# zsummer/zsummerX

Measured on AMD Instinct MI355X. Metric: RC4 GiB/s device-resident (batched session payloads) at 1/2/4/8 MI355X, higher is better.
Workload: dtype u8

## Files before the change

### zsummerx_amd/csrc/zrc4_kernels.hpp

```cpp
#pragma once
#include <hip/hip_runtime.h>
#include <stdint.h>
#include "zrc4_plan.hpp"

namespace zrc4 {

constexpr int kGroupBytes = 256 * 256;

enum : uint32_t {
    kErrSlotRange = 0,
    kErrLdsLayout = 1,
    kErrGroup = 2,
    kErrWords = 4,
};

__device__ __forceinline__ void latch_fault(uint32_t *err, uint32_t kind)
{
    __hip_atomic_store(err + kind, 1u, __ATOMIC_RELAXED, __HIP_MEMORY_SCOPE_SYSTEM);
}

constexpr uint32_t kClaimParts = 64;
struct Claim {
    unsigned long long *word;
    uint32_t epoch;
    const uint32_t *zero;
};

__device__ __forceinline__ unsigned long long claim_part(const Claim &cl, uint32_t g, uint32_t part,
                                                         uint32_t bucket)
{
    return __hip_atomic_exchange(cl.word + (size_t)g * kClaimParts + part,
                                 ((unsigned long long)cl.epoch << 32) | bucket, __ATOMIC_RELAXED,
                                 __HIP_MEMORY_SCOPE_AGENT);
}

__device__ __forceinline__ unsigned long long claim_part_async(const Claim &cl, uint32_t g, uint32_t part,
                                                               uint32_t bucket)
{
    unsigned long long old;
    uint64_t sv;
    const unsigned long long v = ((unsigned long long)cl.epoch << 32) | bucket;
    unsigned long long *addr = cl.word + (size_t)g * kClaimParts + part;
    asm volatile("s_mov_b64 %[sv], exec\n\t"
                 "s_mov_b64 exec, 1\n\t"
                 "global_atomic_swap_x2 %[old], %[a], %[v], off sc0\n\t"
                 "s_mov_b64 exec, %[sv]"
                 : [old] "=&v"(old), [sv] "=&s"(sv)
                 : [a] "v"(addr), [v] "v"(v)
                 : "memory");
    return old;
}

__device__ __forceinline__ unsigned long long claim_part_async_if(const Claim &cl, uint32_t g, uint32_t part,
                                                                  uint32_t bucket, uint32_t pred)
{
    unsigned long long old;
    uint64_t sv;
    const unsigned long long v = ((unsigned long long)cl.epoch << 32) | bucket;
    unsigned long long *addr = cl.word + (size_t)g * kClaimParts + part;
    asm volatile("v_mov_b64 %[old], 0\n\t"
                 "s_cmp_eq_u32 %[p], 0\n\t"
                 "s_cbranch_scc1 CLAIM_SKIP_%=\n\t"
                 "s_mov_b64 %[sv], exec\n\t"
                 "s_mov_b64 exec, 1\n\t"
                 "global_atomic_swap_x2 %[old], %[a], %[v], off sc0\n\t"
                 "s_mov_b64 exec, %[sv]\n\t"
                 "CLAIM_SKIP_%=:"
                 : [old] "=&v"(old), [sv] "=&s"(sv)
                 : [a] "v"(addr), [v] "v"(v), [p] "s"(__builtin_amdgcn_readfirstlane(pred))
                 : "memory", "scc");
    return old;
}

__device__ __forceinline__ void claim_wait(unsigned long long &old)
{
    asm volatile("s_waitcnt vmcnt(0)" : "+v"(old) :: "memory");
}

__device__ __forceinline__ bool claim_lost(const Claim &cl, unsigned long long old)
{
    return (uint32_t)(old >> 32) == cl.epoch;
}

__device__ __forceinline__ bool lds_base_ok(const uint8_t *S, uint32_t *err)
{
    if ((uint32_t)(uintptr_t)S == 0u) return true;
    if (threadIdx.x == 0) latch_fault(err, kErrLdsLayout);
    return false;
}

typedef uint32_t u32x4 __attribute__((ext_vector_type(4)));

__host__ __device__ __forceinline__ uint32_t col_of(uint32_t j)
{
    const uint32_t w = j >> 6, l = j & 63u;
    return ((l & 31u) << 2) | (l >> 5) | ((w & 1u) << 1) | ((w >> 1) << 7);
}

__device__ __forceinline__ uint32_t img_vo(uint32_t j)
{
    return (((j & 127u) >> 3) << 8) | (j & 128u) | ((j & 7u) << 4);
}

#ifndef ZRC4_TIMING
#define ZRC4_TIMING 0
#endif
struct Stamps {
    uint64_t r[4], c[4];
};
__device__ __forceinline__ void stamp(Stamps &s, int i)
{
#if ZRC4_TIMING
    s.r[i] = __builtin_amdgcn_s_memrealtime();
    s.c[i] = __builtin_amdgcn_s_memtime();
#endif
}
constexpr uint32_t kStampBase = 65536u + 16384u;
constexpr uint32_t kStampBytes = 131072u + 16384u + 8192u;
__device__ __forceinline__ void stream_stamp(uint8_t *sink, uint32_t i)
{
#if ZRC4_TIMING
    if ((threadIdx.x & 127u) == 0u && blockIdx.x < 512u && i < 16u) {
        const uint32_t r = blockIdx.x * 2u + (threadIdx.x >> 7);
        uint8_t *b = sink + kStampBase;
        reinterpret_cast<uint64_t *>(b)[r * 16u + i] = __builtin_amdgcn_s_memrealtime();
        if (i == 0u || i == 15u)
            reinterpret_cast<uint64_t *>(b + 131072u)[r * 2u + (i ? 1u : 0u)] = __builtin_amdgcn_s_memtime();
        if (i == 0u) {
            uint32_t hw, xcc;
            asm volatile("s_getreg_b32 %0, hwreg(HW_REG_HW_ID)\n\ts_getreg_b32 %1, hwreg(HW_REG_XCC_ID)"
                         : "=s"(hw), "=s"(xcc));
            uint32_t *o = reinterpret_cast<uint32_t *>(b + 131072u + 16384u) + r * 2u;
            o[0] = hw;
            o[1] = xcc;
        }
    }
#endif
}

__device__ __forceinline__ void stamps_out(const Stamps &s, uint8_t *sink, uint32_t wave)
{
#if ZRC4_TIMING
    if ((threadIdx.x & 63u) == 0u) {
        uint64_t *o = reinterpret_cast<uint64_t *>(sink + ((wave & 1023u) * 64u));
        for (int i = 0; i < 4; ++i) {
            o[i] = s.r[i];
            o[4 + i] = s.c[i];
        }
        uint32_t hw, xcc;
        asm volatile("s_getreg_b32 %0, hwreg(HW_REG_HW_ID)\n\ts_getreg_b32 %1, hwreg(HW_REG_XCC_ID)"
                     : "=s"(hw), "=s"(xcc));
        uint32_t *w = reinterpret_cast<uint32_t *>(sink + 65536u + (wave & 1023u) * 8u);
        w[0] = hw;
        w[1] = xcc;
    }
#endif
}

__device__ __forceinline__ void image_to_lds(uint8_t *lds, const uint8_t *img)
{
    const uint4 *src = reinterpret_cast<const uint4 *>(img);
    uint4 *dst = reinterpret_cast<uint4 *>(lds);
#pragma unroll
    for (int i = 0; i < 16; ++i) dst[i * 256 + threadIdx.x] = src[i * 256 + threadIdx.x];
}

__device__ __forceinline__ void lds_to_image(uint8_t *img, const uint8_t *lds)
{
    const uint4 *src = reinterpret_cast<const uint4 *>(lds);
    uint4 *dst = reinterpret_cast<uint4 *>(img);
#pragma unroll
    for (int i = 0; i < 16; ++i) dst[i * 256 + threadIdx.x] = src[i * 256 + threadIdx.x];
}

__device__ __forceinline__ void gather_column(uint8_t *lds, uint32_t col,
                                              const uint8_t *arena, uint32_t slot)
{
    const uint8_t *img = arena + (size_t)(slot >> 8) * kGroupBytes + col_of(slot & 255u);
    for (int k = 0; k < 256; ++k) lds[(k << 8) | col] = img[k << 8];
}

__device__ __forceinline__ void scatter_column(uint8_t *arena, uint32_t slot,
                                               const uint8_t *lds, uint32_t col)
{
    uint8_t *img = arena + (size_t)(slot >> 8) * kGroupBytes + col_of(slot & 255u);
    for (int k = 0; k < 256; ++k) img[k << 8] = lds[(k << 8) | col];
}

struct Rc4Lane {
    uint32_t x0, a0, ya, ta, x1, col;
};

__device__ __forceinline__ void lane_init(Rc4Lane &st, const uint8_t *S, uint32_t col, uint32_t sxy)
{
    const uint32_t x = sxy & 255u, y = (sxy >> 8) & 255u;
    st.col = col;
    st.x0 = (((x + 1u) & 255u) << 8) | col;
    st.a0 = S[st.x0];
    st.ya = (y << 8) | col;
    st.ta = col;
    st.x1 = col;
}

__device__ __forceinline__ uint16_t lane_xy(const Rc4Lane &st)
{
    return (uint16_t)((((st.x0 >> 8) - 1u) & 255u) | (st.ya & 0xFF00u));
}

__device__ __forceinline__ uint32_t prga_step(uint8_t *S, Rc4Lane &st)
{
    const uint32_t a = st.a0;
    const uint32_t ya = (st.ya & 0xFFu) | ((st.ya + (a << 8)) & 0xFF00u);
    const uint32_t b = S[ya];
    S[ya] = (uint8_t)a;
    const uint32_t xn = (st.x0 & 0xFFu) | ((st.x0 + 256u) & 0xFF00u);
    const uint32_t p = S[xn];
    S[st.x0] = (uint8_t)b;
    const uint32_t k = S[(((a + b) << 8) & 0xFF00u) | st.col];
    st.a0 = p;
    st.x0 = xn;
    st.ya = ya;
    return k;
}

__device__ __forceinline__ uint32_t prga_word(uint8_t *S, Rc4Lane &st)
{
    const uint32_t k0 = prga_step(S, st);
    const uint32_t k1 = prga_step(S, st);
    const uint32_t k2 = prga_step(S, st);
    const uint32_t k3 = prga_step(S, st);
    return k0 | (k1 << 8) | (k2 << 16) | (k3 << 24);
}

__device__ __forceinline__ uint4 xor16(uint8_t *S, Rc4Lane &st, uint4 v)
{
    v.x ^= prga_word(S, st);
    v.y ^= prga_word(S, st);
    v.z ^= prga_word(S, st);
    v.w ^= prga_word(S, st);
    return v;
}

#define ZRC4_CORE(XC, XN, A, P, K)                                                               \
    "v_add_u32_sdwa %[ya], %[ya], %[" #A "] dst_sel:BYTE_1 dst_unused:UNUSED_PRESERVE "          \
    "src0_sel:BYTE_1 src1_sel:BYTE_0\n\t"                                                        \
    "ds_read_u8 %[b], %[ya]\n\t"                                                                 \
    "ds_write_b8 %[ya], %[" #A "]\n\t"                                                           \
    "v_add_u16_e32 %[" #XN "], %[c100], %[" #XC "]\n\t"                                          \
    "ds_read_u8 %[" #P "], %[" #XN "]\n\t"                                                       \
    "s_waitcnt lgkmcnt(2)\n\t"                                                                   \
    "ds_write_b8 %[" #XC "], %[b]\n\t"                                                           \
    "v_add_u32_sdwa %[ta], %[" #A "], %[b] dst_sel:BYTE_1 dst_unused:UNUSED_PRESERVE "           \
    "src0_sel:BYTE_0 src1_sel:BYTE_0\n\t"                                                        \
    "ds_read_u8 %[" #K "], %[ta]\n\t"                                                            \
    "s_waitcnt lgkmcnt(2)\n\t"

#define ZRC4_E ZRC4_CORE(x0, x1, a0, a1, k0)
#define ZRC4_O ZRC4_CORE(x1, x0, a1, a0, k1)

__device__ __forceinline__ void load64(uint4 (&q)[4], const uint4 *p)
{
#pragma unroll
    for (int i = 0; i < 4; ++i) q[i] = p[i];
}

__device__ __forceinline__ uint32_t head_bytes(const uint8_t *msg, uint32_t len)
{
    const uint32_t h = (16u - ((uint32_t)(uintptr_t)msg & 15u)) & 15u;
    return h < len ? h : len;
}

#define ZL_XOR(R, SEL, K)                                                                        \
    "v_xor_b32_sdwa " #R ", " #R ", %[" #K "] dst_sel:" #SEL                                     \
    " dst_unused:UNUSED_PRESERVE src0_sel:" #SEL " src1_sel:BYTE_0\n\t"
#define ZL_MOV(R, SEL, K)                                                                        \
    "v_mov_b32_sdwa " #R ", %[" #K "] dst_sel:" #SEL                                             \
    " dst_unused:UNUSED_PRESERVE src0_sel:BYTE_0\n\t"
#define ZL_W0_(X, D)                                                                             \
    ZRC4_E ZRC4_O X(D, BYTE_0, k0) ZRC4_E X(D, BYTE_1, k1)                                      \
    ZRC4_O X(D, BYTE_2, k0)
#define ZL_W_(X, DP, D)                                                                          \
    ZRC4_E X(DP, BYTE_3, k1) ZRC4_O X(D, BYTE_0, k0)                                            \
    ZRC4_E X(D, BYTE_1, k1) ZRC4_O X(D, BYTE_2, k0)
#define ZL_BLOCK_(X, d0, d1, d2, d3, d4, d5, d6, d7, d8, d9, d10, d11, d12, d13, d14, d15)        \
    ZL_W0_(X, d0) ZL_W_(X, d0, d1) ZL_W_(X, d1, d2) ZL_W_(X, d2, d3) ZL_W_(X, d3, d4)           \
    ZL_W_(X, d4, d5) ZL_W_(X, d5, d6) ZL_W_(X, d6, d7) ZL_W_(X, d7, d8) ZL_W_(X, d8, d9)        \
    ZL_W_(X, d9, d10) ZL_W_(X, d10, d11) ZL_W_(X, d11, d12) ZL_W_(X, d12, d13)                  \
    ZL_W_(X, d13, d14) ZL_W_(X, d14, d15)                                                        \
    "s_waitcnt lgkmcnt(0)\n\t" X(d15, BYTE_3, k1)
#define ZL_BLOCK(...) ZL_BLOCK_(ZL_XOR, __VA_ARGS__)
#define ZL_A0 "v[40:43]"
#define ZL_A1 "v[44:47]"
#define ZL_A2 "v[48:51]"
#define ZL_A3 "v[52:55]"
#define ZL_B0 "v[56:59]"
#define ZL_B1 "v[60:63]"
#define ZL_B2 "v[64:67]"
#define ZL_B3 "v[68:71]"
#define ZL_SRC_DELTA "v_lshl_add_u64 v[90:91], v[90:91], 0, %[dl]\n\t"
#define ZL_PREFETCH_(D, R0, R1, R2, R3)                                                          \
    "s_add_u32 %[i1], %[i], 1\n\t"                                                               \
    "v_cmp_lt_u32_e32 vcc, %[i1], %[nblk]\n\t"                                                   \
    "v_lshl_add_u64 v[90:91], v[88:89], 0, 64\n\t"                                               \
    "v_cndmask_b32_e32 v90, v88, v90, vcc\n\t"                                                   \
    "v_cndmask_b32_e32 v91, v89, v91, vcc\n\t"                                                   \
    D                                                                                            \
    "global_load_dwordx4 " R0 ", v[90:91], off\n\t"                                              \
    "global_load_dwordx4 " R1 ", v[90:91], off offset:16\n\t"                                    \
    "global_load_dwordx4 " R2 ", v[90:91], off offset:32\n\t"                                    \
    "global_load_dwordx4 " R3 ", v[90:91], off offset:48\n\t"
#define ZL_STORE(R0, R1, R2, R3)                                                                 \
    "global_store_dwordx4 v[88:89], " R0 ", off\n\t"                                             \
    "global_store_dwordx4 v[88:89], " R1 ", off offset:16\n\t"                                   \
    "global_store_dwordx4 v[88:89], " R2 ", off offset:32\n\t"                                   \
    "global_store_dwordx4 v[88:89], " R3 ", off offset:48\n\t"                                   \
    "v_lshl_add_u64 v[88:89], v[88:89], 0, 64\n\t"                                               \
    "s_add_u32 %[i], %[i], 1\n\t"
#define ZL_ACTIVE                                                                                \
    "v_cmp_lt_u32_e32 vcc, %[i], %[nblk]\n\t"                                                    \
    "s_and_b64 exec, exec, vcc\n\t"                                                              \
    "s_cbranch_execz ZL_DONE_%=\n\t"
#define ZL_HALF_A_(D)                                                                            \
    ZL_ACTIVE                                                                                    \
    ZL_PREFETCH_(D, ZL_B0, ZL_B1, ZL_B2, ZL_B3)                                                  \
    "s_waitcnt vmcnt(8)\n\t"                                                                     \
    ZL_BLOCK(v40, v41, v42, v43, v44, v45, v46, v47, v48, v49, v50, v51, v52, v53, v54, v55)    \
    ZL_STORE(ZL_A0, ZL_A1, ZL_A2, ZL_A3)
#define ZL_HALF_B_(D)                                                                            \
    ZL_ACTIVE                                                                                    \
    ZL_PREFETCH_(D, ZL_A0, ZL_A1, ZL_A2, ZL_A3)                                                  \
    "s_waitcnt vmcnt(8)\n\t"                                                                     \
    ZL_BLOCK(v56, v57, v58, v59, v60, v61, v62, v63, v64, v65, v66, v67, v68, v69, v70, v71)    \
    ZL_STORE(ZL_B0, ZL_B1, ZL_B2, ZL_B3)
#define ZL_FIRST_(D)                                                                             \
    "s_mov_b32 %[i], 0\n\t"                                                                      \
    ZL_PREFETCH_(D, ZL_B0, ZL_B1, ZL_B2, ZL_B3)                                                  \
    "v_mov_b32 v72, 0\n\tv_mov_b32 v73, 0\n\tv_mov_b32 v74, 0\n\tv_mov_b32 v75, 0\n\t"             \
    "v_mov_b32 v76, 0\n\tv_mov_b32 v77, 0\n\tv_mov_b32 v78, 0\n\tv_mov_b32 v79, 0\n\t"             \
    "v_mov_b32 v80, 0\n\tv_mov_b32 v81, 0\n\tv_mov_b32 v82, 0\n\tv_mov_b32 v83, 0\n\t"             \
    "v_mov_b32 v84, 0\n\tv_mov_b32 v85, 0\n\tv_mov_b32 v86, 0\n\tv_mov_b32 v87, 0\n\t"             \
    ZL_BLOCK(v72, v73, v74, v75, v76, v77, v78, v79, v80, v81, v82, v83, v84, v85, v86, v87)    \
    "s_waitcnt vmcnt(4)\n\t"                                                                     \
    "v_xor_b32_e32 v40, v40, v72\n\tv_xor_b32_e32 v41, v41, v73\n\t"                               \
    "v_xor_b32_e32 v42, v42, v74\n\tv_xor_b32_e32 v43, v43, v75\n\t"                               \
    "v_xor_b32_e32 v44, v44, v76\n\tv_xor_b32_e32 v45, v45, v77\n\t"                               \
    "v_xor_b32_e32 v46, v46, v78\n\tv_xor_b32_e32 v47, v47, v79\n\t"                               \
    "v_xor_b32_e32 v48, v48, v80\n\tv_xor_b32_e32 v49, v49, v81\n\t"                               \
    "v_xor_b32_e32 v50, v50, v82\n\tv_xor_b32_e32 v51, v51, v83\n\t"                               \
    "v_xor_b32_e32 v52, v52, v84\n\tv_xor_b32_e32 v53, v53, v85\n\t"                               \
    "v_xor_b32_e32 v54, v54, v86\n\tv_xor_b32_e32 v55, v55, v87\n\t"                               \
    ZL_STORE(ZL_A0, ZL_A1, ZL_A2, ZL_A3)                                                         \
    "s_branch ZL_MID_%=\n\t"

#define ZL_HALF_A ZL_HALF_A_("")
#define ZL_HALF_B ZL_HALF_B_("")
#define ZL_FIRST ZL_FIRST_("")

__device__ __forceinline__ void crypt_blocks_asm(Rc4Lane &st, uint4 *&p, uint32_t nblk,
                                                 const uint4 (&A)[4])
{
    u32x4 a0 = {A[0].x, A[0].y, A[0].z, A[0].w}, a1 = {A[1].x, A[1].y, A[1].z, A[1].w};
    u32x4 a2 = {A[2].x, A[2].y, A[2].z, A[2].w}, a3 = {A[3].x, A[3].y, A[3].z, A[3].w};
    u32x4 b0, b1, b2, b3, q0, q1, q2, q3;
    uint64_t pa = (uint64_t)(uintptr_t)p, pn, save;
    uint32_t i, i1, b, k0, k1, a1s;
    asm volatile(
        "s_mov_b64 %[save], exec\n\t"
        ZL_FIRST
        "ZL_LOOP_%=:\n\t"
        ZL_HALF_A
        "ZL_MID_%=:\n\t"
        ZL_HALF_B
        "s_branch ZL_LOOP_%=\n\t"
        "ZL_DONE_%=:\n\t"
        "s_mov_b64 exec, %[save]\n\t"
        : [ya] "+v"(st.ya), [ta] "+v"(st.ta), [x0] "+v"(st.x0), [x1] "+v"(st.x1),
          [a0] "+v"(st.a0), [a1] "=&v"(a1s), [b] "=&v"(b), [k0] "=&v"(k0), [k1] "=&v"(k1),
          "+{v[88:89]}"(pa), "=&{v[90:91]}"(pn), [i] "=&s"(i), [i1] "=&s"(i1), [save] "=&s"(save),
          "+{v[40:43]}"(a0), "+{v[44:47]}"(a1), "+{v[48:51]}"(a2), "+{v[52:55]}"(a3),
          "=&{v[56:59]}"(b0), "=&{v[60:63]}"(b1), "=&{v[64:67]}"(b2), "=&{v[68:71]}"(b3),
          "=&{v[72:75]}"(q0), "=&{v[76:79]}"(q1), "=&{v[80:83]}"(q2), "=&{v[84:87]}"(q3)
        : [nblk] "v"(nblk), [c100] "s"(0x100u)
        : "memory", "vcc", "scc");
    p = reinterpret_cast<uint4 *>((uintptr_t)pa);
}

#define ZL_TO_LOOP(TAILWAIT)                                                                     \
    asm volatile(                                                                                \
        "s_mov_b64 %[save], exec\n\t"                                                            \
        ZL_FIRST_(ZL_SRC_DELTA)                                                                  \
        "ZL_LOOP_%=:\n\t"                                                                        \
        ZL_HALF_A_(ZL_SRC_DELTA)                                                                 \
        "ZL_MID_%=:\n\t"                                                                         \
        ZL_HALF_B_(ZL_SRC_DELTA)                                                                 \
        "s_branch ZL_LOOP_%=\n\t"                                                                \
        "ZL_DONE_%=:\n\t"                                                                        \
        "s_mov_b64 exec, %[save]\n\t"                                                            \
        TAILWAIT                                                                                 \
        : [ya] "+v"(st.ya), [ta] "+v"(st.ta), [x0] "+v"(st.x0), [x1] "+v"(st.x1),                \
          [a0] "+v"(st.a0), [a1] "=&v"(a1s), [b] "=&v"(b), [k0] "=&v"(k0), [k1] "=&v"(k1),       \
          "+{v[88:89]}"(pa), "=&{v[90:91]}"(pn), [i] "=&s"(i), [i1] "=&s"(i1), [save] "=&s"(save), \
          "+{v[40:43]}"(a0), "+{v[44:47]}"(a1), "+{v[48:51]}"(a2), "+{v[52:55]}"(a3),            \
          "=&{v[56:59]}"(b0), "=&{v[60:63]}"(b1), "=&{v[64:67]}"(b2), "=&{v[68:71]}"(b3),        \
          "=&{v[72:75]}"(q0), "=&{v[76:79]}"(q1), "=&{v[80:83]}"(q2), "=&{v[84:87]}"(q3)         \
        : [nblk] "v"(nblk), [c100] "s"(0x100u), [dl] "v"(delta)                                  \
        : "memory", "vcc", "scc")
template <bool DRAIN = false>
__device__ __forceinline__ void crypt_blocks_to_asm(Rc4Lane &st, uint4 *&p, uint32_t nblk, const uint4 (&A)[4],
                                                    uint64_t delta)
{
    u32x4 a0 = {A[0].x, A[0].y, A[0].z, A[0].w}, a1 = {A[1].x, A[1].y, A[1].z, A[1].w};
    u32x4 a2 = {A[2].x, A[2].y, A[2].z, A[2].w}, a3 = {A[3].x, A[3].y, A[3].z, A[3].w};
    u32x4 b0, b1, b2, b3, q0, q1, q2, q3;
    uint64_t pa = (uint64_t)(uintptr_t)p, pn, save;
    uint32_t i, i1, b, k0, k1, a1s;
    if constexpr (DRAIN)
        ZL_TO_LOOP("s_waitcnt vmcnt(4)\n\t");
    else
        ZL_TO_LOOP("");
    p = reinterpret_cast<uint4 *>((uintptr_t)pa);
}
#undef ZL_TO_LOOP

#define ZL_KS_HALF(T0, T1, T2, T3, ...)                                                          \
    ZL_ACTIVE                                                                                    \
    "s_waitcnt vmcnt(4)\n\t"                                                                     \
    ZL_BLOCK_(ZL_MOV, __VA_ARGS__)                                                               \
    ZL_STORE(T0, T1, T2, T3)
__device__ __forceinline__ void keystream_blocks_asm(Rc4Lane &st, uint4 *&p, uint32_t nblk)
{
    u32x4 a0, a1, a2, a3, b0, b1, b2, b3;
    uint64_t pa = (uint64_t)(uintptr_t)p, save;
    uint32_t i, b, k0, k1, a1s;
    asm volatile(
        "s_mov_b64 %[save], exec\n\t"
        "s_mov_b32 %[i], 0\n\t"
        "ZL_LOOP_%=:\n\t"
        ZL_KS_HALF(ZL_A0, ZL_A1, ZL_A2, ZL_A3, v40, v41, v42, v43, v44, v45, v46, v47, v48, v49, v50, v51, v52,
                   v53, v54, v55)
        ZL_KS_HALF(ZL_B0, ZL_B1, ZL_B2, ZL_B3, v56, v57, v58, v59, v60, v61, v62, v63, v64, v65, v66, v67, v68,
                   v69, v70, v71)
        "s_branch ZL_LOOP_%=\n\t"
        "ZL_DONE_%=:\n\t"
        "s_mov_b64 exec, %[save]\n\t"
        : [ya] "+v"(st.ya), [ta] "+v"(st.ta), [x0] "+v"(st.x0), [x1] "+v"(st.x1),
          [a0] "+v"(st.a0), [a1] "=&v"(a1s), [b] "=&v"(b), [k0] "=&v"(k0), [k1] "=&v"(k1),
          "+{v[88:89]}"(pa), [i] "=&s"(i), [save] "=&s"(save),
          "=&{v[40:43]}"(a0), "=&{v[44:47]}"(a1), "=&{v[48:51]}"(a2), "=&{v[52:55]}"(a3),
          "=&{v[56:59]}"(b0), "=&{v[60:63]}"(b1), "=&{v[64:67]}"(b2), "=&{v[68:71]}"(b3)
        : [nblk] "v"(nblk), [c100] "s"(0x100u)
        : "memory", "vcc", "scc");
    p = reinterpret_cast<uint4 *>((uintptr_t)pa);
}

__device__ __forceinline__ void issue_block_asm(uint4 (&A)[4], const uint8_t *msg)
{
    u32x4 a0, a1, a2, a3;
// ... 2355 lines not shown
```

### zsummerx_amd/csrc/zrc4_win.hpp

```cpp
#pragma once
#include "zrc4_kernels.hpp"
#include "zrc4_plan.hpp"

namespace zrc4 {

constexpr uint32_t kWinLanes = 16;
constexpr uint32_t kWinStreams = 4;
constexpr uint32_t kWinRing = 2048;
constexpr uint32_t kWinUnits = kWinRing / 16 / kWinLanes;
#ifndef ZRC4_WIN_TAG_LIMIT
#define ZRC4_WIN_TAG_LIMIT (1u << 23)
#endif
constexpr uint32_t kWinTagLimit = ZRC4_WIN_TAG_LIMIT;

struct WinLane {
    uint32_t xa;
    uint32_t y;
    uint32_t v;
    uint32_t rp;
};

#define ZW_ADDR(XA)                                                                               \
    "v_add_u32_sdwa v106, " XA ", %[l] dst_sel:BYTE_0 dst_unused:UNUSED_PRESERVE src0_sel:DWORD "  \
    "src1_sel:DWORD\n\t"
__device__ __forceinline__ void win_windows(WinLane &w, uint32_t rem, uint32_t l, uint32_t sb, uint32_t mb,
                                            uint32_t rb)
{
    const uint32_t bitl = 1u << l, l1 = (l + 1) << 8;
    asm volatile(
        "s_mov_b64 s[46:47], 0\n\t"
        "v_and_b32 v120, 0xff, %[y]\n\t"
        "s_mov_b64 s[44:45], 0\n\t"
        "v_mov_b32 v123, 0\n\t"
        "v_mov_b32 v106, %[sb]\n\t"
        "v_mov_b32 v126, %[sb]\n\t"
        ZW_ADDR("%[xa]")
        "ds_read_u8 v107, v106\n\t"
        "ZW_LOOP_%=:\n\t"
        "s_waitcnt lgkmcnt(0)\n\t"
        "v_add_u32_dpp v112, v107, v107 row_shr:1 row_mask:0xf bank_mask:0xf bound_ctrl:0\n\t"
        "v_max_u32_dpp v120, v120, v120 quad_perm:[1,0,3,2] row_mask:0xf bank_mask:0xf\n\t"
        "v_cmp_ge_u32_e64 s[42:43], v123, %[v]\n\t"
        "v_add_u32_dpp v112, v112, v112 row_shr:2 row_mask:0xf bank_mask:0xf\n\t"
        "v_max_u32_dpp v120, v120, v120 quad_perm:[2,3,0,1] row_mask:0xf bank_mask:0xf\n\t"
        "v_add_u32 %[v], 0x100, %[v]\n\t"
        "v_add_u32_dpp v112, v112, v112 row_shr:4 row_mask:0xf bank_mask:0xf\n\t"
        "v_max_u32_dpp v120, v120, v120 row_half_mirror row_mask:0xf bank_mask:0xf\n\t"
        "s_or_b64 s[42:43], s[42:43], s[44:45]\n\t"
        "v_cndmask_b32_e64 v124, v121, v122, s[42:43]\n\t"
        "v_add_u32_dpp v112, v112, v112 row_shr:8 row_mask:0xf bank_mask:0xf\n\t"
        "v_max_u32_dpp v120, v120, v120 row_mirror row_mask:0xf bank_mask:0xf\n\t"
        "v_add_u32 v112, v112, v120\n\t"
        "v_add_u32_sdwa v114, %[sb], v112 dst_sel:DWORD dst_unused:UNUSED_PAD src0_sel:DWORD src1_sel:BYTE_0\n\t"
        "v_and_b32 v112, 0xff, v112\n\t"
        "v_lshl_add_u32 v115, v112, 2, %[mb]\n\t"
        "ds_read_u8 v116, v114\n\t"
        "ds_max_u32 v115, %[v]\n\t"
        "ds_read_b32 v117, v115\n\t"
        "s_mov_b64 s[40:41], exec\n\t"
        "s_mov_b64 exec, s[46:47]\n\t"
        "ds_write_b8 v125, v124\n\t"
        "s_mov_b64 exec, s[40:41]\n\t"
        "v_and_b32 %[y], 0xff, v120\n\t"
        "v_sub_u32 v118, v112, %[xa]\n\t"
        "v_and_b32 v118, 0xff, v118\n\t"
        "v_med3_u32 v119, v118, %[l], 16\n\t"
        "v_cmp_ne_u32 vcc, v118, %[l]\n\t"
        "v_cndmask_b32 v119, 16, v119, vcc\n\t"
        "v_lshlrev_b32 v118, v119, 1\n\t"
        "v_min_u32 v119, 16, %[rem]\n\t"
        "v_lshlrev_b32 v119, v119, 1\n\t"
        "v_or_b32 v118, v118, v119\n\t"
        "v_or_b32 v119, v118, %[bitl]\n\t"
        "v_or_b32 v130, %[l1], v112\n\t"
        "v_bfi_b32 v125, %[rmask], %[rp], %[rb]\n\t"
        "s_waitcnt lgkmcnt(1)\n\t"
        "v_cmp_ne_u32 vcc, v117, %[v]\n\t"
        "v_cndmask_b32 v118, v118, v119, vcc\n\t"
        "v_add_u32_sdwa v126, v107, v116 dst_sel:BYTE_0 dst_unused:UNUSED_PRESERVE src0_sel:DWORD src1_sel:DWORD\n\t"
        "v_add_u32 v128, v107, v116\n\t"
        "ds_read_u8 v121, v126\n\t"
        "v_or_b32_dpp v118, v118, v118 quad_perm:[1,0,3,2] row_mask:0xf bank_mask:0xf\n\t"
        "v_sub_u32 v131, v128, %[xa]\n\t"
        "v_and_b32 v128, 0xff, v128\n\t"
        "v_or_b32_dpp v118, v118, v118 quad_perm:[2,3,0,1] row_mask:0xf bank_mask:0xf\n\t"
        "v_and_b32 v131, 0xff, v131\n\t"
        "v_lshl_add_u32 v129, v128, 2, %[mb]\n\t"
        "v_or_b32_dpp v118, v118, v118 row_half_mirror row_mask:0xf bank_mask:0xf\n\t"
        "v_cmp_le_u32_e64 s[44:45], v131, %[l]\n\t"
        "v_mov_b32 v131, v106\n\t"
        "v_or_b32_dpp v118, v118, v118 row_mirror row_mask:0xf bank_mask:0xf\n\t"
        "v_ffbl_b32 v118, v118\n\t"
        "v_cmp_lt_u32 vcc, %[l], v118\n\t"
        "v_add_u32_sdwa v106, v106, v118 dst_sel:BYTE_0 dst_unused:UNUSED_PRESERVE src0_sel:BYTE_0 src1_sel:DWORD\n\t"
        "s_and_saveexec_b64 s[40:41], vcc\n\t"
        "ds_write_b8 v131, v116\n\t"
        "ds_write_b8 v114, v107\n\t"
        "s_mov_b64 exec, s[40:41]\n\t"
        "ds_read_u8 v107, v106\n\t"
        "ds_read_u8 v122, v126\n\t"
        "ds_read_b32 v123, v129\n\t"
        "s_and_b64 s[46:47], vcc, s[40:41]\n\t"
        "v_cndmask_b32 v120, %[y], v130, vcc\n\t"
        "v_add_u32 %[xa], %[xa], v118\n\t"
        "v_and_b32 %[xa], 0xff, %[xa]\n\t"
        "v_sub_u32 %[rem], %[rem], v118\n\t"
        "v_add_u32 %[rp], %[rp], v118\n\t"
        "v_cmp_ne_u32 vcc, 0, %[rem]\n\t"
        "s_cbranch_vccnz ZW_LOOP_%=\n\t"
        "s_waitcnt lgkmcnt(0)\n\t"
        "v_max_u32_dpp v120, v120, v120 quad_perm:[1,0,3,2] row_mask:0xf bank_mask:0xf\n\t"
        "v_cmp_ge_u32_e64 s[42:43], v123, %[v]\n\t"
        "s_or_b64 s[42:43], s[42:43], s[44:45]\n\t"
        "v_cndmask_b32_e64 v124, v121, v122, s[42:43]\n\t"
        "v_max_u32_dpp v120, v120, v120 quad_perm:[2,3,0,1] row_mask:0xf bank_mask:0xf\n\t"
        "s_nop 1\n\t"
        "v_max_u32_dpp v120, v120, v120 row_half_mirror row_mask:0xf bank_mask:0xf\n\t"
        "s_nop 1\n\t"
        "v_max_u32_dpp v120, v120, v120 row_mirror row_mask:0xf bank_mask:0xf\n\t"
        "s_mov_b64 s[40:41], exec\n\t"
        "s_mov_b64 exec, s[46:47]\n\t"
        "ds_write_b8 v125, v124\n\t"
        "s_mov_b64 exec, s[40:41]\n\t"
        "v_and_b32 %[y], 0xff, v120\n\t"
        "s_waitcnt lgkmcnt(0)\n\t"
        : [xa] "+v"(w.xa), [y] "+v"(w.y), [v] "+v"(w.v), [rem] "+v"(rem), [rp] "+v"(w.rp)
        : [l] "v"(l), [sb] "v"(sb), [mb] "v"(mb), [rb] "v"(rb), [bitl] "v"(bitl), [l1] "v"(l1),
          [rmask] "s"(kWinRing - 1)
        : "memory", "vcc", "scc", "v106", "v107", "v112", "v114", "v115", "v116", "v117", "v118", "v119", "v120",
          "v121", "v122", "v123", "v124", "v125", "v126", "v128", "v129", "v130", "v131", "s40", "s41",
          "s42", "s43", "s44", "s45", "s46", "s47");
}

struct WinGroups {
    uint32_t g[kWinMaxBuckets];
};

template <int MODE, bool FRAME, bool DECL = false, int IO = kIoInPlace>
__global__ void __launch_bounds__(64)
crypt_win_kernel(uint8_t *__restrict__ arena, uint16_t *__restrict__ xy, const uint32_t *__restrict__ ids,
                 uint32_t first_slot, uint8_t *__restrict__ payload, const uint64_t *__restrict__ off,
                 const uint32_t *__restrict__ len, uint32_t n, uint32_t capacity, uint32_t *__restrict__ err,
                 uint8_t *__restrict__ sink, AuxArgs<IO> fr, Claim cl, WinGroups dg = WinGroups{})
{
    constexpr bool KS = IO == kIoKs, TO = IO == kIoTo;
    static_assert(!(KS || TO) || !FRAME, "the write-only and out-of-place forms are never framed");
    Stamps ts;
    stamp(ts, 0);
    __shared__ __attribute__((aligned(1024))) uint32_t Mk[kWinStreams * 256];
    __shared__ __attribute__((aligned(kWinRing))) uint8_t Ring[kWinStreams * kWinRing];
    __shared__ __attribute__((aligned(256))) uint8_t Sb[kWinStreams * 256];

    const uint32_t k = blockIdx.x, xcd = k & 7u, idx = k >> 3;
    const bool local = ((gridDim.x >> 6) & 7u) == 0u;
    const uint32_t q = local ? (idx & 63u) : ((idx & 7u) | (xcd << 3));
    const uint32_t wg = local ? (((idx >> 6) << 3) | xcd) : (idx >> 3);
    const uint32_t lane = threadIdx.x, l = lane & 15u, b = lane >> 4;
    const uint32_t kb = ((q >> 5) << 7) + (q & 31u) + 32u * b;
    uint32_t slot, L = 0, ent = 0;
    uint64_t O = 0, SO = 0;
    bool valid;
    uint32_t rows[4];
    uint32_t sxy, sxy_g;
    unsigned long long cold = 0;
    uint32_t gclaim = 0;
    bool bad = false;
    if constexpr (MODE == kRange) {
        const uint32_t e = wg * kGroup + kb;
        ent = e;
        slot = first_slot + e;
        valid = e < n;
        if (!__builtin_amdgcn_ballot_w64(valid)) return;
        const uint8_t *img = arena + (size_t)(slot >> 8) * kGroupBytes + 4u * q;
#pragma unroll
        for (int r = 0; r < 4; ++r)
            rows[r] = *reinterpret_cast<const uint32_t *>(img + (size_t)(lane + 64u * r) * 256u);
        if (valid) {
            L = len[e];
            O = off[e];
            if constexpr (TO) SO = fr.src_off[e];
        }
        sxy = valid ? xy[slot] : 0u;
    } else {
        uint32_t *te = reinterpret_cast<uint32_t *>(Ring);
        uint32_t *tl = te + 256;
        uint64_t *to = reinterpret_cast<uint64_t *>(Ring + 2048);
        uint32_t *fl = reinterpret_cast<uint32_t *>(Ring + 4096);
        uint64_t *tso = reinterpret_cast<uint64_t *>(Ring + 6144);
        static_assert(kWinStreams * kWinRing >= 8192, "the slot tables use the ring's 8 KiB");
        uint32_t idq[4], lq[4];
        uint64_t oq[4], soq[4];
        bool bq[4];
        uint32_t gw = ZRC4_INVALID;
#pragma unroll
        for (int r = 0; r < 4; ++r) {
            const uint32_t e = wg * kGroup + lane + 64u * r;
            const bool v = e < n;
            idq[r] = v ? ids[e] : ZRC4_INVALID;
            lq[r] = v ? len[e] : 0u;
            oq[r] = v ? off[e] : 0u;
            if constexpr (TO) soq[r] = v ? fr.src_off[e] : 0u;
        }
        if constexpr (DECL) {
            gw = dg.g[wg];
            const uint32_t gl = gw != ZRC4_INVALID ? gw : 0u;
            const uint8_t *img = arena + (size_t)gl * kGroupBytes + 4u * q;
#pragma unroll
            for (int r = 0; r < 4; ++r)
                rows[r] = *reinterpret_cast<const uint32_t *>(img + (size_t)(lane + 64u * r) * 256u);
            sxy_g = xy[gl * 256u + kb];
        }
#pragma unroll
        for (int r = 0; r < 4; ++r) te[lane + 64u * r] = ZRC4_INVALID;
#pragma unroll
        for (int r = 0; r < 4; ++r) {
            if (idq[r] >= capacity && idq[r] != ZRC4_INVALID) {
                latch_fault(err, kErrSlotRange);
                idq[r] = ZRC4_INVALID;
            }
            bq[r] = idq[r] != ZRC4_INVALID && lq[r] != 0u;
        }
        if (lane < 9) fl[lane] = 0u;
        if constexpr (!DECL) {
#pragma unroll
            for (int r = 3; r >= 0; --r) {
                const uint64_t bm = __builtin_amdgcn_ballot_w64(bq[r]);
                if (bm) gw = __builtin_amdgcn_readlane(idq[r], (int)__builtin_ctzll(bm)) >> 8;
            }
        }
        if constexpr (FRAME) {
#pragma unroll
            for (int r = 0; r < 4; ++r) {
                const uint32_t e = wg * kGroup + lane + 64u * r;
                if (lane == q && e < n && !bq[r])
                    frame_walk(payload + fr.off[e], fr.len[e], fr.bound, fr.maxp, e, fr.npk, fr.used, fr.status,
                               fr.pkt_len);
            }
        }
        if (gw == ZRC4_INVALID) {
            if constexpr (DECL) {
                const bool busy = __builtin_amdgcn_ballot_w64(bq[0] | bq[1] | bq[2] | bq[3]) != 0ull;
                if (busy && q == 0u && lane == 0) latch_fault(err, kErrGroup);
            }
            return;
        }
        if constexpr (!DECL) {
            gw = __builtin_amdgcn_readfirstlane(gw);
            const uint8_t *img = arena + (size_t)gw * kGroupBytes + 4u * q;
#pragma unroll
            for (int r = 0; r < 4; ++r)
                rows[r] = *reinterpret_cast<const uint32_t *>(img + (size_t)(lane + 64u * r) * 256u);
            sxy_g = xy[gw * 256u + kb];
        }
        gclaim = gw;
        __syncthreads();
#pragma unroll
        for (int r = 0; r < 4; ++r) {
            if (bq[r]) {
                const uint32_t kk = idq[r] & 255u;
                if ((idq[r] >> 8) != gw) fl[8] = 1u;
                if (atomicOr(&fl[kk >> 5], 1u << (kk & 31u)) & (1u << (kk & 31u))) fl[8] = 1u;
                te[kk] = wg * kGroup + lane + 64u * r;
                tl[kk] = lq[r];
                to[kk] = oq[r];
                if constexpr (TO) tso[kk] = soq[r];
            }
        }
        __syncthreads();
        slot = gw * 256u + kb;
        ent = te[kb];
        valid = ent != ZRC4_INVALID;
        if (valid) {
            L = tl[kb];
            O = to[kb];
            if constexpr (TO) SO = tso[kb];
        }
        bad = fl[8] != 0u;
    }
    uint8_t *img = arena + (size_t)(slot >> 8) * kGroupBytes + 4u * q;
    uint8_t *msg = payload + O;
    const uint8_t *smsg = msg;
    if constexpr (TO) smsg = fr.src + SO;
    const bool aligned = (((uintptr_t)msg | (uintptr_t)smsg) & 15u) == 0u;

#define ZRC4_WIN_FILL                                                                       \
    do {                                                                                    \
        _Pragma("unroll") for (int r = 0; r < 4; ++r) {                                     \
            const uint32_t kk = lane + 64u * r;                                             \
            _Pragma("unroll") for (uint32_t s4 = 0; s4 < 4; ++s4) {                         \
                const uint8_t v = (uint8_t)(rows[r] >> (8 * s4));                           \
                Sb[s4 * 256u + kk] = v;                                                     \
            }                                                                               \
        }                                                                                   \
        _Pragma("unroll") for (int i = 0; i < 4; ++i)                                       \
            reinterpret_cast<uint4 *>(Mk)[lane + 64 * i] = make_uint4(0, 0, 0, 0);         \
    } while (0)
    if constexpr (MODE == kGrouped) {
        if (bad) {
            claim_wait(cold);
            if (lane == 0) latch_fault(err, kErrGroup);
            return;
        }
        sxy = valid ? sxy_g : 0u;
        if (!__builtin_amdgcn_ballot_w64(valid)) {
            claim_wait(cold);
            return;
        }
        ZRC4_WIN_FILL;
    }

    uint4 pre[kWinUnits];
    if constexpr (!KS) {
#pragma unroll
        for (uint32_t u = 0; u < kWinUnits; ++u) {
            const uint32_t pos = 16u * (l + kWinLanes * u);
            if constexpr (MODE == kGrouped)
                pre[u] = *reinterpret_cast<const uint4 *>(aligned && pos + 16u <= L ? smsg + pos : sink + 16u * lane);
            else if (aligned && pos + 16u <= L)
                pre[u] = *reinterpret_cast<const uint4 *>(smsg + pos);
        }
    }
    if constexpr (MODE == kGrouped) cold = claim_part_async(cl, gclaim, q, wg);

    uint8_t *S = Sb + b * 256u;
    uint32_t *M = Mk + b * 256u;
    uint8_t *R = Ring + b * kWinRing;
    if constexpr (MODE != kGrouped) ZRC4_WIN_FILL;
#undef ZRC4_WIN_FILL
    __syncthreads();
    stamp(ts, 1);

    const uint32_t sb = (uint32_t)(uintptr_t)S, mb = (uint32_t)(uintptr_t)M, rb = (uint32_t)(uintptr_t)R;
    WinLane w{((sxy & 0xFFu) + 1u) & 0xFFu, sxy >> 8, (1u << 8) | (255u - l), l};

    for (uint32_t c0 = 0; __builtin_amdgcn_ballot_w64(c0 < L); c0 += kWinRing) {
        const uint32_t c1 = L < c0 + kWinRing ? L : c0 + kWinRing;
        const uint32_t rem = c0 < L ? c1 - c0 : 0u;
        if (w.v >= (kWinTagLimit << 8)) {
#pragma unroll
            for (int i = 0; i < 4; ++i) reinterpret_cast<uint4 *>(Mk)[lane + 64 * i] = make_uint4(0, 0, 0, 0);
            w.v = (1u << 8) | (255u - l);
        }
        win_windows(w, rem, l, sb, mb, rb);
        if constexpr (MODE == kGrouped) {
            if (c0 == 0u) {
                claim_wait(cold);
                if (claim_lost(cl, ((unsigned long long)__builtin_amdgcn_readfirstlane((uint32_t)(cold >> 32))) << 32)) {
                    if (lane == 0) latch_fault(err, kErrGroup);
                    return;
                }
            }
        }
        if (c0 >= L) {
        } else if constexpr (KS) {
            if (aligned) {
#pragma unroll
                for (uint32_t u = 0; u < kWinUnits; ++u) {
                    const uint32_t pos = c0 + 16u * (l + kWinLanes * u);
                    if (pos + 16u <= c1)
                        *reinterpret_cast<uint4 *>(msg + pos) =
                            *reinterpret_cast<const uint4 *>(R + (pos & (kWinRing - 1u)));
                }
                const uint32_t tpos = c0 + ((c1 - c0) & ~15u) + l;
                if (tpos < c1) msg[tpos] = R[tpos & (kWinRing - 1u)];
            } else {
                for (uint32_t pos = c0 + l; pos < c1; pos += kWinLanes) msg[pos] = R[pos & (kWinRing - 1u)];
            }
        } else if (aligned) {
#pragma unroll
            for (uint32_t u = 0; u < kWinUnits; ++u) {
                const uint32_t pos = c0 + 16u * (l + kWinLanes * u);
                if (pos + 16u <= c1) {
                    const uint4 ks = *reinterpret_cast<const uint4 *>(R + (pos & (kWinRing - 1u)));
                    uint4 v = pre[u];
                    v.x ^= ks.x; v.y ^= ks.y; v.z ^= ks.z; v.w ^= ks.w;
                    *reinterpret_cast<uint4 *>(msg + pos) = v;
                }
            }
            const uint32_t tpos = c0 + ((c1 - c0) & ~15u) + l;
            if constexpr (TO) {
                if (tpos < c1) msg[tpos] = smsg[tpos] ^ R[tpos & (kWinRing - 1u)];
            } else {
                if (tpos < c1) msg[tpos] ^= R[tpos & (kWinRing - 1u)];
            }
        } else if constexpr (TO) {
            for (uint32_t pos = c0 + l; pos < c1; pos += kWinLanes) msg[pos] = smsg[pos] ^ R[pos & (kWinRing - 1u)];
        } else {
            for (uint32_t pos = c0 + l; pos < c1; pos += kWinLanes) msg[pos] ^= R[pos & (kWinRing - 1u)];
        }
        if constexpr (!KS) {
            const uint32_t n0 = c0 + kWinRing;
#pragma unroll
            for (uint32_t u = 0; u < kWinUnits; ++u) {
                const uint32_t pos = n0 + 16u * (l + kWinLanes * u);
                if (aligned && pos + 16u <= L) pre[u] = *reinterpret_cast<const uint4 *>(smsg + pos);
            }
        }
    }

    stamp(ts, 2);
    if (valid && l == 0) xy[slot] = (uint16_t)(((w.xa - 1u) & 0xFFu) | ((w.y & 0xFFu) << 8));
    if constexpr (FRAME) {
        __builtin_amdgcn_s_waitcnt(0);
        if (valid && l == 0)
            frame_walk(payload + fr.off[ent], fr.len[ent], fr.bound, fr.maxp, ent, fr.npk, fr.used, fr.status,
                       fr.pkt_len);
    }
    __syncthreads();
#pragma unroll
    for (int r = 0; r < 4; ++r) {
        const uint32_t kk = lane + 64u * r;
        const uint32_t v = (uint32_t)Sb[kk] | ((uint32_t)Sb[256u + kk] << 8) | ((uint32_t)Sb[512u + kk] << 16) |
                           ((uint32_t)Sb[768u + kk] << 24);
        *reinterpret_cast<uint32_t *>(img + (size_t)kk * 256u) = v;
    }
#if ZRC4_TIMING
    __builtin_amdgcn_s_waitcnt(0);
    stamp(ts, 3);
    stamps_out(ts, sink, wg * 64u + q);
#else
    (void)sink;
#endif
}

}
```

Baseline: 157.2.

## Hoist range-mode metadata loads and overlap LDS init with image row fetch

```diff
diff --git a/zsummerx_amd/csrc/zrc4_kernels.hpp b/zsummerx_amd/csrc/zrc4_kernels.hpp
--- a/zsummerx_amd/csrc/zrc4_kernels.hpp
+++ b/zsummerx_amd/csrc/zrc4_kernels.hpp
@@ -107,12 +107,19 @@
 #endif
 struct Stamps {
     uint64_t r[4], c[4];
+    uint64_t m[2] = {0, 0};
 };
 __device__ __forceinline__ void stamp(Stamps &s, int i)
 {
 #if ZRC4_TIMING
     s.r[i] = __builtin_amdgcn_s_memrealtime();
     s.c[i] = __builtin_amdgcn_s_memtime();
+#endif
+}
+__device__ __forceinline__ void stamp_mid(Stamps &s, int i)
+{
+#if ZRC4_TIMING
+    s.m[i] = __builtin_amdgcn_s_memtime();
 #endif
 }
 constexpr uint32_t kStampBase = 65536u + 16384u;
@@ -153,6 +160,9 @@
         uint32_t *w = reinterpret_cast<uint32_t *>(sink + 65536u + (wave & 1023u) * 8u);
         w[0] = hw;
         w[1] = xcc;
+        uint32_t *m = reinterpret_cast<uint32_t *>(sink + 65536u + 8192u + (wave & 1023u) * 8u);
+        m[0] = s.m[0] ? (uint32_t)(s.m[0] - s.c[0]) : 0u;
+        m[1] = s.m[1] ? (uint32_t)(s.m[1] - s.c[0]) : 0u;
     }
 #endif
 }
diff --git a/zsummerx_amd/csrc/zrc4_win.hpp b/zsummerx_amd/csrc/zrc4_win.hpp
--- a/zsummerx_amd/csrc/zrc4_win.hpp
+++ b/zsummerx_amd/csrc/zrc4_win.hpp
@@ -166,21 +166,39 @@
     uint32_t gclaim = 0;
     bool bad = false;
     if constexpr (MODE == kRange) {
+        asm volatile("" ::"s"(arena), "s"(xy), "s"(first_slot), "s"(payload), "s"(off), "s"(len), "s"(n), "s"(sink),
+                     "s"(gridDim.x));
+        if constexpr (TO) asm volatile("" ::"s"(fr.src), "s"(fr.src_off));
+        const uint32_t sb = (uint32_t)(uintptr_t)(Sb + b * 256u), mb = (uint32_t)(uintptr_t)(Mk + b * 256u),
+                       rb = (uint32_t)(uintptr_t)(Ring + b * kWinRing);
+        const uint32_t bitl = 1u << l, l1 = (l + 1) << 8, tag0 = (1u << 8) | (255u - l), pos0 = 16u * l;
+#define ZRC4_WIN_EARLY                                                                      \
+    do {                                                                                    \
+        _Pragma("unroll") for (int i = 0; i < 4; ++i)                                       \
+            reinterpret_cast<uint4 *>(Mk)[lane + 64 * i] = make_uint4(0, 0, 0, 0);         \
+        asm volatile("" ::"v"(sb), "v"(mb), "v"(rb), "v"(bitl), "v"(l1), "v"(tag0), "v"(pos0)); \
+        _Pragma("unroll") for (uint32_t u = 1; u < kWinUnits; ++u)                          \
+            asm volatile("" ::"v"(pos0 + 16u * kWinLanes * u));    \
+        __builtin_amdgcn_sched_barrier(0);                                                  \
+    } while (0)
         const uint32_t e = wg * kGroup + kb;
         ent = e;
         slot = first_slot + e;
         valid = e < n;
-        if (!__builtin_amdgcn_ballot_w64(valid)) return;
+        const uint32_t ec = valid ? e : n - 1u;
+        const uint32_t Lq = len[ec];
+        O = off[ec];
+        if constexpr (TO) SO = fr.src_off[ec];
+        const uint16_t sq = xy[first_slot + ec];
+        __builtin_amdgcn_sched_barrier(0);
         const uint8_t *img = arena + (size_t)(slot >> 8) * kGroupBytes + 4u * q;
 #pragma unroll
         for (int r = 0; r < 4; ++r)
             rows[r] = *reinterpret_cast<const uint32_t *>(img + (size_t)(lane + 64u * r) * 256u);
-        if (valid) {
-            L = len[e];
-            O = off[e];
-            if constexpr (TO) SO = fr.src_off[e];
-        }
-        sxy = valid ? xy[slot] : 0u;
+        ZRC4_WIN_EARLY;
+        if (!__builtin_amdgcn_ballot_w64(valid)) return;
+        L = valid ? Lq : 0u;
+        sxy = valid ? (uint32_t)sq : 0u;
     } else {
         uint32_t *te = reinterpret_cast<uint32_t *>(Ring);
         uint32_t *tl = te + 256;
@@ -292,9 +310,20 @@
                 Sb[s4 * 256u + kk] = v;                                                     \
             }                                                                               \
         }                                                                                   \
-        _Pragma("unroll") for (int i = 0; i < 4; ++i)                                       \
-            reinterpret_cast<uint4 *>(Mk)[lane + 64 * i] = make_uint4(0, 0, 0, 0);         \
+        if constexpr (MODE == kGrouped) {                                                   \
+            _Pragma("unroll") for (int i = 0; i < 4; ++i)                                   \
+                reinterpret_cast<uint4 *>(Mk)[lane + 64 * i] = make_uint4(0, 0, 0, 0);     \
+        }                                                                                   \
     } while (0)
+#if ZRC4_TIMING
+#define ZRC4_WIN_STAMP_IN                                                                   \
+    do {                                                                                    \
+        asm volatile("" ::"v"(rows[0]), "v"(rows[1]), "v"(rows[2]), "v"(rows[3]));          \
+        stamp_mid(ts, 0);                                                                   \
+    } while (0)
+#else
+#define ZRC4_WIN_STAMP_IN (void)0
+#endif
     if constexpr (MODE == kGrouped) {
         if (bad) {
             claim_wait(cold);
@@ -306,18 +335,27 @@
             claim_wait(cold);
             return;
         }
+        ZRC4_WIN_STAMP_IN;
         ZRC4_WIN_FILL;
     }
 
     uint4 pre[kWinUnits];
-    if constexpr (!KS) {
+    if constexpr (!KS && MODE == kGrouped) {
 #pragma unroll
         for (uint32_t u = 0; u < kWinUnits; ++u) {
             const uint32_t pos = 16u * (l + kWinLanes * u);
-            if constexpr (MODE == kGrouped)
-                pre[u] = *reinterpret_cast<const uint4 *>(aligned && pos + 16u <= L ? smsg + pos : sink + 16u * lane);
-            else if (aligned && pos + 16u <= L)
-                pre[u] = *reinterpret_cast<const uint4 *>(smsg + pos);
+            pre[u] = *reinterpret_cast<const uint4 *>(aligned && pos + 16u <= L ? smsg + pos : sink + 16u * lane);
+        }
+    } else if constexpr (!KS) {
+        const uint32_t pos0 = 16u * l;
+        const bool any = aligned && pos0 + 16u <= L;
+        const uint32_t full = (L - pos0 - 16u) / (16u * kWinLanes);
+        const uint32_t last = any ? 16u * kWinLanes * full : 0u;
+        const uint8_t *base = any ? smsg + pos0 : sink + 16u * lane;
+#pragma unroll
+        for (uint32_t u = 0; u < kWinUnits; ++u) {
+            const uint32_t d = 16u * kWinLanes * u;
+            pre[u] = *reinterpret_cast<const uint4 *>(base + (d < last ? d : last));
         }
     }
     if constexpr (MODE == kGrouped) cold = claim_part_async(cl, gclaim, q, wg);
@@ -325,8 +363,15 @@
     uint8_t *S = Sb + b * 256u;
     uint32_t *M = Mk + b * 256u;
     uint8_t *R = Ring + b * kWinRing;
-    if constexpr (MODE != kGrouped) ZRC4_WIN_FILL;
+    if constexpr (MODE != kGrouped) {
+        asm volatile("" ::"v"(((sxy & 0xFFu) + 1u) & 0xFFu), "v"(sxy >> 8));
+        __builtin_amdgcn_sched_barrier(0);
+        ZRC4_WIN_STAMP_IN;
+        ZRC4_WIN_FILL;
+    }
 #undef ZRC4_WIN_FILL
+#undef ZRC4_WIN_EARLY
+#undef ZRC4_WIN_STAMP_IN
     __syncthreads();
     stamp(ts, 1);
 
@@ -341,6 +386,9 @@
             for (int i = 0; i < 4; ++i) reinterpret_cast<uint4 *>(Mk)[lane + 64 * i] = make_uint4(0, 0, 0, 0);
             w.v = (1u << 8) | (255u - l);
         }
+#if ZRC4_TIMING
+        if (c0 == 0u) stamp_mid(ts, 1);
+#endif
         win_windows(w, rem, l, sb, mb, rb);
         if constexpr (MODE == kGrouped) {
             if (c0 == 0u) {
```

Result: faster. 159.8 (median of 6 runs) (+1.7%).
